# faltiska/Matcha-TTS-24k

Hardware: AMD Instinct MI355X
Metric: mel-frames/s (100-bin, 24 kHz) end-to-end synthesise(), n_timesteps=10 (higher is better)
Workload: dtype f32 via 2-term f16 split (fp32 accumulate); 1 GPU; configs[1]: batch=32 random phoneme seqs len=128, n_spks=1, euler n_timesteps=10, fp32, prod v20 architecture, random-init weights, T_pad=640 / 320 valid frames per utterance (reference 2x padding kept in the results; the estimator folds the identical padded frames, DESIGN.md section 4), noise from the device seed-42 generator; per_gpu_batch=32, global_batch=32, parallelism=dp1, n_feats=100

## Files before the change

### include/mtts.h

```cpp
#ifndef MTTS_H
#define MTTS_H

#include <stddef.h>
#include <stdint.h>

#ifdef __cplusplus
extern "C" {
#endif

#define MTTS_ABI_VERSION 2
#define MTTS_IMAGE_REVISION 6

typedef struct mtts_ctx mtts_ctx;

typedef struct mtts_config {
    int32_t n_feats;
    int32_t n_spks;
    int32_t spk_emb_dim;
    int32_t n_vocab;
    int32_t enc_channels;
    int32_t enc_filter;
    int32_t enc_heads;
    int32_t enc_layers;
    int32_t enc_kernel;
// ... 74 lines not shown
                  int a_nparts, const float* d_w,
                  void* d_wpacked, const float* d_bias, int N, int act, const float* d_p0, const float* d_p1,
                  const float* d_res, int ldr, const float* d_out_mask, float out_scale, float* d_out, int ldc,
                  float* d_stats_out, int terms, void* stream);

int64_t mtts_gemm_p16_scratch_bytes(int B, int T_in, int C, int T_out, int N);
int mtts_gemm_p16(const float* d_a, int lda, int B, int T_in, int C, int ntaps, const int* h_tap_off, int in_stride, int T_out,
                  const float* d_a_mask, const float* d_a_mean, const float* d_a_rstd, const float* d_a_part, int a_nparts,
                  const float* d_w, void* d_wpacked, const float* d_bias, int N, int act, const float* d_p0, const float* d_p1,
                  const float* d_res, int ldr, const float* d_out_mask, float out_scale, float* d_out, int ldc,
                  float* d_out16_f32, float out_lscale, float* d_stats_out, int force_bm, void* d_scratch, void* stream);

int64_t mtts_conv_gn_scratch_bytes(int B, int T, int C, int N);
int mtts_conv_gn(const float* d_x, int B, int T, int C, int c1, const float* d_w, void* d_wpacked, const float* d_bias, int N,
                 const float* d_gamma, const float* d_beta, const float* d_mask, const float* d_chbias, const int* d_nrows,
                 const int* d_nextra, const float* d_bias_stats, float eps, float* d_out, void* d_scratch, void* stream);

int mtts_attention_f32(const float* d_qkv, const float* d_mask, int B, int T, int H, int D, float scale, int mask_mode,
                       float* d_out, void* stream);

int mtts_attention_p16(const float* d_qkv, const float* d_mask, int B, int T, int H, int D, float scale, int mask_mode,
                       float* d_out, void* d_scratch, void* stream);

int64_t mtts_chain_stream_frags(int C, int inner, int ch, int n_qkv);
int mtts_chain_plan(int M, int ch, int* qb, int* prefetch_wgs);
int mtts_chain_stream_pack(int C, int inner, int ch, int n_qkv, const float* h_w_out, const float* h_w1, const float* h_w2,
                           const float* h_w_qkv, uint16_t* h_dst);
int64_t mtts_chain_stream_frags_pair(int C, int inner, int ch, int n_qkv);
int mtts_chain_stream_pack_pair(int C, int inner, int ch, int n_qkv, const float* h_w_out, const float* h_w1, const float* h_w2,
                                const float* h_w_qkv, uint16_t* h_dst);
int64_t mtts_tblock_chain_scratch_bytes(int M, int C, int inner, int n_qkv, int ch);
int mtts_tblock_chain(const float* d_att, const float* d_x, int M, int C, int inner, const float* h_w_out, const float* h_b_out,
                      const float* h_w1, const float* h_b1, const float* h_p0, const float* h_p1, const float* h_w2,
                      const float* h_b2, const float* h_w_qkv, const float* h_b_qkv, int n_qkv, const float* d_out_mask, int qb,
                      int ch, float* d_x_out, float* d_qkv_out, void* d_scratch, void* stream);
int mtts_tblock_chain_timed(const float* d_att, const float* d_x, int M, int C, int inner, const float* h_w_out, const float* h_b_out,
                            const float* h_w1, const float* h_b1, const float* h_p0, const float* h_p1, const float* h_w2,
                            const float* h_b2, const float* h_w_qkv, const float* h_b_qkv, int n_qkv, const float* d_out_mask,
                            int qb, int ch, float* d_x_out, float* d_qkv_out, void* d_scratch, void* stream, int repeat, float* h_ms);
int mtts_tblock_chain_pair_timed(const float* d_att, const float* d_x, int M, int C, int inner, const float* h_w_out, const float* h_b_out,
                                 const float* h_w1, const float* h_b1, const float* h_p0, const float* h_p1, const float* h_w2,
                                 const float* h_b2, const float* h_w_qkv, const float* h_b_qkv, int n_qkv, const float* d_out_mask,
                                 int qb, int ch, float* d_x_out, float* d_qkv_out, void* d_scratch, void* stream, int repeat, float* h_ms);

int64_t mtts_chain_stream_frags_h16(int C, int inner, int ch, int n_qkv);
int mtts_chain_stream_pack_h16(int C, int inner, int ch, int n_qkv, const float* h_w_out, const float* h_w1, const float* h_w2,
// ... 90 lines not shown
```

### matcha-tts-24k_amd/_hip.py

```python
from __future__ import annotations

import ctypes as C
import os
import subprocess
from pathlib import Path
from typing import Dict, Optional

import numpy as np
import torch

from .hparams import PathHParams

HERE = Path(__file__).resolve().parent
CSRC = HERE / "csrc"
LIB = Path(os.environ["MTTS_HIP_LIB"]) if os.environ.get("MTTS_HIP_LIB") else HERE / "libmtts_hip.so"
SOURCES = ["gemm_f32.hip", "attention_f32.hip", "gemm_p16.hip", "tblock_chain.hip", "tblock_chain_h16.hip", "resnet_conv.hip", "norm_glue.hip", "vocos.hip", "waveform.hip", "mel_frontend.hip", "style_encoder.hip", "mas.hip", "model.hip", "pack.hip", "decoder.hip", "encoder.hip", "unit_entries.hip"]
HEADERS = [CSRC / "kernels.h", CSRC / "device_utils.h", CSRC / "model.h", CSRC / "host.h", HERE.parent / "include" / "mtts.h"]
SOLVERS = {"euler": 0, "midpoint": 1, "rk4": 2}


class MttsConfig(C.Structure):
    _fields_ = [(n, C.c_int32) for n in (
        "n_feats", "n_spks", "spk_emb_dim", "n_vocab", "enc_channels", "enc_filter", "enc_heads", "enc_layers",
        "enc_kernel", "prenet_layers", "prenet_kernel", "dp_filter", "dp_kernel", "dp_layers", "dec_levels")] + [
# ... 87 lines not shown
        "mtts_import_weights": (i32, [vp, vp, i64, i32]),
        "mtts_encoder_workspace_bytes": (i64, [vp, i32, i32]),
        "mtts_text_encoder_forward": (i32, [vp, vp, vp, vp, vp, i32, i32, vp, vp, vp, vp, i64, vp]),
        "mtts_speaker_embedding": (i32, [vp, i32, vp, i32, vp, vp]),
        "mtts_durations": (i32, [vp, vp, f32, f32, i32, i32, vp, vp, vp, vp]),
        "mtts_durations_per_utterance": (i32, [vp, vp, vp, vp, i32, i32, vp, vp, vp, vp]),
        "mtts_durations_given": (i32, [vp, vp, f32, vp, vp, i32, i32, vp, vp, vp, vp]),
        "mtts_align_pool": (i32, [vp, vp, vp, i32, i32, i32, i32, vp, vp, vp, vp]),
        "mtts_set_frame_limits": (i32, [vp, vp]),
        "mtts_decoder_workspace_bytes": (i64, [vp, i32, i32]),
        "mtts_decoder_forward": (i32, [vp, vp, vp, vp, f32, i32, i32, vp, vp, i64, vp]),
        "mtts_cfm_solve": (i32, [vp, vp, vp, vp, i32, vp, i32, i32, i32, i32, vp, i32, f32, f32, vp, i64, vp]),
        "mtts_fold_rows": (i32, [vp, i32, i32]),
        "mtts_cfm_solve_folded": (i32, [vp, vp, vp, vp, i32, i32, vp, i32, i32, i32, i32, i32, vp, i32, f32, f32, vp, i64, vp]),
        "mtts_gemm_packed_bytes": (i64, [i32, i32, i32]),
        "mtts_attention_p16": (i32, [vp, vp, i32, i32, i32, i32, f32, i32, vp, vp, vp]),
        "mtts_gemm_p16_scratch_bytes": (i64, [i32, i32, i32, i32, i32]),
        "mtts_conv_gn_scratch_bytes": (i64, [i32, i32, i32, i32]),
        "mtts_conv_gn": (i32, [vp, i32, i32, i32, i32, vp, vp, vp, i32, vp, vp, vp, vp, vp, vp, vp, f32, vp, vp, vp]),
        "mtts_gemm_p16": (i32, [vp, i32, i32, i32, i32, i32, vp, i32, i32, vp, vp, vp, vp, i32, vp, vp, vp, i32, i32, vp, vp, vp,
                                i32, vp, f32, vp, i32, vp, f32, vp, i32, vp, vp]),
        "mtts_gemm_f32": (i32, [vp, i32, i32, i32, i32, i32, vp, i32, i32, vp, vp, vp, vp, i32, vp, vp, vp, i32, i32, vp, vp, vp,
                                i32, vp, f32, vp, i32, vp, i32, vp]),
        "mtts_attention_f32": (i32, [vp, vp, i32, i32, i32, i32, f32, i32, vp, vp]),
        "mtts_chain_stream_frags": (i64, [i32, i32, i32, i32]),
        "mtts_chain_plan": (i32, [i32, i32, C.POINTER(C.c_int), C.POINTER(C.c_int)]),
        "mtts_chain_stream_frags_pair": (i64, [i32, i32, i32, i32]),
        "mtts_chain_stream_pack_pair": (i32, [i32, i32, i32, i32, vp, vp, vp, vp, vp]),
        "mtts_chain_stream_pack": (i32, [i32, i32, i32, i32, vp, vp, vp, vp, vp]),
        "mtts_tblock_chain_scratch_bytes": (i64, [i32, i32, i32, i32, i32]),
        "mtts_tblock_chain": (i32, [vp, vp, i32, i32, i32, vp, vp, vp, vp, vp, vp, vp, vp, vp, vp, i32, vp, i32, i32, vp, vp, vp, vp]),
        "mtts_tblock_chain_timed": (i32, [vp, vp, i32, i32, i32, vp, vp, vp, vp, vp, vp, vp, vp, vp, vp, i32, vp, i32, i32, vp, vp, vp, vp,
                                          i32, C.POINTER(C.c_float)]),
        "mtts_tblock_chain_pair_timed": (i32, [vp, vp, i32, i32, i32, vp, vp, vp, vp, vp, vp, vp, vp, vp, vp, i32, vp, i32, i32, vp, vp, vp, vp,
                                          i32, C.POINTER(C.c_float)]),
        "mtts_chain_stream_frags_h16": (i64, [i32, i32, i32, i32]),
        "mtts_chain_stream_pack_h16": (i32, [i32, i32, i32, i32, vp, vp, vp, vp, i32, vp, C.POINTER(C.c_int)]),
        "mtts_tblock_chain_h16_scratch_bytes": (i64, [i32, i32, i32, i32, i32]),
        "mtts_tblock_chain_h16": (i32, [vp, vp, i32, i32, i32, vp, vp, vp, vp, vp, vp, vp, vp, vp, vp, i32, vp, i32, i32, i32, i32, vp, vp, vp, vp]),
        "mtts_tblock_chain_h16_timed": (i32, [vp, vp, i32, i32, i32, vp, vp, vp, vp, vp, vp, vp, vp, vp, vp, i32, vp, i32, i32, i32, i32, vp, vp, vp, vp,
                                              i32, C.POINTER(C.c_float)]),
        "mtts_row_stats": (i32, [vp, i32, i32, i32, f32, vp, vp, vp]),
        "mtts_channel_layernorm": (i32, [vp, i32, i32, i32, vp, vp, f32, i32, vp, vp, vp, vp]),
        "mtts_groupnorm_scratch_bytes": (i64, [i32, i32, i32]),
        "mtts_groupnorm_mish": (i32, [vp, vp, vp, vp, i32, i32, i32, i32, f32, vp, vp, vp]),
        "mtts_vocos_create": (vp, [i32, i32, i32, i32, i32, i32]),
# ... 599 lines not shown
                                          n_qkv, ptr(out_mask), int(bool(bf16)), qb, ch, pf_wgs, ptr(x_out), ptr(qkv), scratch.data_ptr(),
                                          stream_ptr(), repeat, C.byref(ms)))
    torch.cuda.synchronize()
    if repeat:
        return x_out, qkv, ms.value
    return x_out, qkv


def attention_f32(qkv, mask, B, T, H, D, scale, mask_mode):
    lib = load()
    out = torch.empty(B * T, H * D, dtype=torch.float32, device=qkv.device)
    check(lib.mtts_attention_f32(ptr(qkv), ptr(mask), B, T, H, D, float(scale), mask_mode, ptr(out), stream_ptr()))
    return out


def attention_p16(qkv, mask, B, T, H, D, scale, mask_mode):
    lib = load()
    out = torch.empty(B * T, H * D, dtype=torch.float32, device=qkv.device)
    scratch = torch.empty(16 * B * T * H * D, dtype=torch.uint8, device=qkv.device)
    check(lib.mtts_attention_p16(ptr(qkv), ptr(mask), B, T, H, D, float(scale), mask_mode, ptr(out), scratch.data_ptr(), stream_ptr()))
    return out


def row_stats(x, eps=1e-5):
    lib = load()
    M, Cc = x.shape
    mean = torch.empty(M, dtype=torch.float32, device=x.device)
    rstd = torch.empty(M, dtype=torch.float32, device=x.device)
    check(lib.mtts_row_stats(ptr(x), M, Cc, Cc, eps, ptr(mean), ptr(rstd), stream_ptr()))
    return mean, rstd


def channel_layernorm(x, gamma, beta, B, T, *, act=0, film=None, mask=None, eps=1e-5):
    lib = load()
    y = torch.empty_like(x)
    check(lib.mtts_channel_layernorm(ptr(x), B, T, x.shape[1], ptr(gamma), ptr(beta), float(eps), act, ptr(film), ptr(mask), ptr(y),
                                     stream_ptr()))
    return y


def groupnorm_mish(y, gamma, beta, mask, B, T, G=8, eps=1e-5):
    lib = load()
    Cc = y.shape[1]
    scratch = torch.empty(lib.mtts_groupnorm_scratch_bytes(B, T, G), dtype=torch.uint8, device=y.device)
    out = torch.empty_like(y)
    check(lib.mtts_groupnorm_mish(ptr(y), ptr(gamma), ptr(beta), ptr(mask), B, T, Cc, G, eps, ptr(out), scratch.data_ptr(),
# ... 3 lines not shown
```

### matcha-tts-24k_amd/csrc/attention_f32.hip

```cpp
#include "kernels.h"
#include "device_utils.h"
#include <cstdlib>
#include <string>

namespace mtts {

using f32x16 = __attribute__((ext_vector_type(16))) float;
using f32x4 = __attribute__((ext_vector_type(4))) float;
using f16x8 = __attribute__((ext_vector_type(8))) _Float16;
using f16x4 = __attribute__((ext_vector_type(4))) _Float16;

constexpr int AT_QW = 32;
constexpr int AT_K = 64;
constexpr int AT_D = 64;
constexpr int AT_KS = 72;
constexpr float NEG_BIG = -1e30f;
constexpr float LOG2E = 1.44269504088896340736f;

__device__ __forceinline__ f16x4 tr_read4(const _Float16* lds_ptr) {
    typedef __fp16 h4 __attribute__((__vector_size__(4 * sizeof(__fp16))));
    const h4 v = __builtin_amdgcn_ds_read_tr16_b64_v4f16((__attribute__((address_space(3))) h4*)(lds_ptr));
    return __builtin_bit_cast(f16x4, v);
}

using bf16x8_a = __attribute__((ext_vector_type(8))) __bf16;
template <bool BF>
__device__ __forceinline__ f32x16 att_mfma(f16x8 a, f16x8 b, f32x16 c) {
    if constexpr (BF) return __builtin_amdgcn_mfma_f32_32x32x16_bf16(__builtin_bit_cast(bf16x8_a, a), __builtin_bit_cast(bf16x8_a, b), c, 0, 0, 0);
    else return __builtin_amdgcn_mfma_f32_32x32x16_f16(a, b, c, 0, 0, 0);
}
template <int NW, bool P16, bool ONE = false, bool HALF = false, bool BF = false, int KR = AT_K>
__global__ __launch_bounds__(64 * NW, KR > AT_K ? 1 : 2) void attention_f32_kernel(const AttnArgs p) {
    static_assert(!HALF || (P16 && ONE), "H16 I/O runs the single-product loop");
    static_assert(!BF || HALF, "bfloat16 planes exist in the 16-bit storage mode only");
    constexpr bool WHOLE = KR > AT_K;
    constexpr int NT = 64 * NW;
    constexpr int SROWS = NT / 4;
    constexpr int SP = KR / SROWS;
    static_assert(SP >= 1 && SP * SROWS == KR && (!WHOLE || NW * AT_QW >= KR), "staging passes cover the rows held");
    __shared__ __attribute__((aligned(16))) _Float16 Ks[2 * KR * AT_KS];
    __shared__ __attribute__((aligned(16))) _Float16 Vs[2 * 2 * KR * 32];
    __shared__ __attribute__((aligned(16))) float Bs[KR];

    const int tid = threadIdx.x, lane = tid & 63, wave = tid >> 6;
    const int lq = lane & 31, h = lane >> 5;
    const int qblocks = (p.T + NW * AT_QW - 1) / (NW * AT_QW);
    int swz;
    {
        const int nwg = gridDim.x, id = blockIdx.x;
        const int xcd = id & 7, q = nwg >> 3, r = nwg & 7;
        swz = (xcd < r ? xcd * (q + 1) : r * (q + 1) + (xcd - r) * q) + (id >> 3);
    }
    const int qb = swz % qblocks, head = (swz / qblocks) % p.H, b = swz / (qblocks * p.H);
    const int q0 = qb * (NW * AT_QW) + wave * AT_QW;
    const int ld = 3 * p.H * p.D;
    const size_t rowbase = (size_t)b * p.T;
    const int Tb = p.klen ? min(p.T, p.klen[b]) : p.T;
    const float* qptr = p.qkv + head * p.D;
    const float* kptr = p.qkv + p.H * p.D + head * p.D;
    const float* vptr = p.qkv + 2 * p.H * p.D + head * p.D;
    const float ninf = -__builtin_huge_valf();

    const int qi = q0 + lq;
    const bool q_in = qi < p.T;
    const float scale2 = p.scale * LOG2E;
    f16x8 qh[4], ql[4];
    const _Float16* q16 = p.qkv16 + head * ((HALF ? 1 : 2) * AT_D);
    const _Float16* k16 = q16 + (HALF ? 1 : 2) * p.H * AT_D;
    const _Float16* v16 = q16 + (HALF ? 2 : 4) * p.H * AT_D;
    if constexpr (P16) {
        const _Float16* qrow = q16 + (rowbase + (q_in ? qi : 0)) * (size_t)p.ld16;
#pragma unroll
        for (int kb = 0; kb < 4; ++kb) {
            const f16x8 z = {0, 0, 0, 0, 0, 0, 0, 0};
            const _Float16* src = HALF ? qrow + 16 * kb + 8 * h : qrow + (kb >> 1) * 64 + (kb & 1) * 16 + 8 * h;
            qh[kb] = q_in ? *reinterpret_cast<const f16x8*>(src) : z;
            ql[kb] = (q_in && !HALF) ? *reinterpret_cast<const f16x8*>(src + 32) : z;
        }
    } else
#pragma unroll
    for (int kb = 0; kb < 4; ++kb) {
#pragma unroll
        for (int half4 = 0; half4 < 2; ++half4) {
            f32x4 v = {0.f, 0.f, 0.f, 0.f};
            const int d = 16 * kb + 8 * h + 4 * half4;
            if (q_in && d < p.D) v = *reinterpret_cast<const f32x4*>(qptr + (rowbase + qi) * ld + d);
#pragma unroll
            for (int e = 0; e < 4; ++e) {
                const _Float16 a = (_Float16)v[e];
                qh[kb][4 * half4 + e] = a;
                ql[kb][4 * half4 + e] = (_Float16)(v[e] - (float)a);
            }
        }
    }

    f32x16 o[2];
#pragma unroll
    for (int t = 0; t < 2; ++t)
#pragma unroll
        for (int r = 0; r < 16; ++r) o[t][r] = 0.f;
    float m_run = NEG_BIG, l_run = 0.f;

    const int srow = tid >> 2;
    const int sd = (tid & 3) * 4;
    f32x4 rk[SP][4], rv[SP][4];
    float rbias[SP];
    bool r_in[SP];
    auto fetch = [&](int k0) {
#pragma unroll
        for (int sp = 0; sp < SP; ++sp) {
            const int key = k0 + srow + SROWS * sp;
            r_in[sp] = key < Tb;
            const size_t row = rowbase + (r_in[sp] ? key : 0);
#pragma unroll
            for (int c = 0; c < 4; ++c) {
                if constexpr (HALF) {
                    if (c < 2) {
                        rk[sp][c] = *reinterpret_cast<const f32x4*>(k16 + row * p.ld16 + ((tid & 3) + 4 * c) * 8);
// ... 48 lines not shown
                *reinterpret_cast<f16x4*>(Ks + r * AT_KS + sd + 16 * c) = kh;
                *reinterpret_cast<f16x4*>(Ks + KR * AT_KS + r * AT_KS + sd + 16 * c) = kl;
                const f32x4 vv = ok ? rv[sp][c] : zero;
                f16x4 vh4, vl4;
#pragma unroll
                for (int e = 0; e < 4; ++e) {
                    const _Float16 a = (_Float16)vv[e];
                    vh4[e] = a;
                    vl4[e] = (_Float16)(vv[e] - (float)a);
                }
                const int dcol = sd + 16 * c;
                *reinterpret_cast<f16x4*>(Vs + ((dcol >> 5) * KR + r) * 32 + (dcol & 31)) = vh4;
                *reinterpret_cast<f16x4*>(Vs + ((2 + (dcol >> 5)) * KR + r) * 32 + (dcol & 31)) = vl4;
            }
            if ((tid & 3) == 0) {
                float bv = ninf;
                if (r_in[sp]) bv = (p.mask_mode == 0) ? rbias[sp] * LOG2E : (rbias[sp] != 0.f ? 0.f : ninf);
                Bs[r] = bv;
            }
        }
    };

    const int ntiles = (Tb + AT_K - 1) / AT_K;
    fetch(0);
    if constexpr (WHOLE) {
        stage();
        __syncthreads();
    }
    for (int kt = 0; kt < ntiles; ++kt) {
        const int kbase = WHOLE ? kt * AT_K : 0;
        if constexpr (!WHOLE) {
            if (kt) __syncthreads();
            stage();
            __syncthreads();
            if (kt + 1 < ntiles) fetch((kt + 1) * AT_K);
        }

        f32x16 s[2];
#pragma unroll
        for (int t = 0; t < 2; ++t) {
#pragma unroll
            for (int r = 0; r < 16; ++r) s[t][r] = 0.f;
            const _Float16* kp = Ks + (kbase + 32 * t + lq) * AT_KS + 8 * h;
#pragma unroll
            for (int kb = 0; kb < 4; ++kb) {
                const f16x8 kh = *reinterpret_cast<const f16x8*>(kp + 16 * kb);
                const f16x8 kl = *reinterpret_cast<const f16x8*>(kp + KR * AT_KS + 16 * kb);
                if constexpr (!ONE) {
                    s[t] = __builtin_amdgcn_mfma_f32_32x32x16_f16(kl, qh[kb], s[t], 0, 0, 0);
                    s[t] = __builtin_amdgcn_mfma_f32_32x32x16_f16(kh, ql[kb], s[t], 0, 0, 0);
                }
                s[t] = att_mfma<BF>(kh, qh[kb], s[t]);
            }
        }
        float mx = NEG_BIG;
#pragma unroll
        for (int t = 0; t < 2; ++t)
#pragma unroll
            for (int g4 = 0; g4 < 4; ++g4) {
                const f32x4 bb = *reinterpret_cast<const f32x4*>(Bs + kbase + 32 * t + 8 * g4 + 4 * h);
#pragma unroll
                for (int e = 0; e < 4; ++e) {
                    const float v = fmaf(s[t][4 * g4 + e], scale2, bb[e]);
                    s[t][4 * g4 + e] = v;
                    mx = fmaxf(mx, v);
                }
            }
        mx = fmaxf(mx, __shfl_xor(mx, 32));
        const float m_new = fmaxf(m_run, mx);
        const float alpha = __builtin_amdgcn_exp2f(m_run - m_new);
        float psum = 0.f;
#pragma unroll
        for (int t = 0; t < 2; ++t)
#pragma unroll
            for (int r = 0; r < 16; ++r) {
                const float pv = __builtin_amdgcn_exp2f(s[t][r] - m_new);
                s[t][r] = pv;
                psum += pv;
            }
        l_run = l_run * alpha + psum;
        if (__any(m_new != m_run)) {
#pragma unroll
            for (int t = 0; t < 2; ++t)
#pragma unroll
                for (int r = 0; r < 16; ++r) o[t][r] *= alpha;
        }
        m_run = m_new;
#pragma unroll
        for (int t = 0; t < 2; ++t)
#pragma unroll
            for (int ks = 0; ks < 2; ++ks) {
                f16x8 ph, pl;
                if constexpr (BF) {
                    using u32x4 = __attribute__((ext_vector_type(4))) unsigned int;
                    u32x4 w;
#pragma unroll
                    for (int j = 0; j < 4; ++j) w[j] = pack_bf16(s[t][8 * ks + 2 * j], s[t][8 * ks + 2 * j + 1]);
                    ph = __builtin_bit_cast(f16x8, w);
                    pl = ph;
                } else {
#pragma unroll
                    for (int j = 0; j < 8; ++j) {
                        const float pv = s[t][8 * ks + j];
                        const _Float16 a = (_Float16)pv;
                        ph[j] = a;
                        pl[j] = (_Float16)(pv - (float)a);
                    }
                }
                const int k0 = 32 * t + 16 * ks + 4 * h;
#pragma unroll
                for (int dt = 0; dt < 2; ++dt) {
                    const _Float16* vp = Vs + ((dt * KR) + kbase + k0 + ((lane & 15) >> 2)) * 32 + 16 * ((lane >> 4) & 1) + 4 * (lane & 3);
                    f16x8 vh, vl;
                    const f16x4 h0 = tr_read4(vp), h1 = tr_read4(vp + 8 * 32);
                    const f16x4 l0 = tr_read4(vp + 2 * KR * 32), l1 = tr_read4(vp + 2 * KR * 32 + 8 * 32);
#pragma unroll
                    for (int e = 0; e < 4; ++e) { vh[e] = h0[e]; vh[4 + e] = h1[e]; vl[e] = l0[e]; vl[4 + e] = l1[e]; }
                    if constexpr (!ONE) {
                        o[dt] = __builtin_amdgcn_mfma_f32_32x32x16_f16(vl, ph, o[dt], 0, 0, 0);
                        o[dt] = __builtin_amdgcn_mfma_f32_32x32x16_f16(vh, pl, o[dt], 0, 0, 0);
                    }
                    o[dt] = att_mfma<BF>(vh, ph, o[dt]);
                }
            }
    }

    const float l_tot = l_run + __shfl_xor(l_run, 32);
    const float inv = l_tot > 0.f ? 1.0f / l_tot : 0.f;
    bool range_bad = false;
    if (P16) {
        if (q_in) {
            _Float16* op = p.out16 + (rowbase + qi) * (size_t)p.ldo16 + head * ((HALF ? 1 : 2) * AT_D);
#pragma unroll
            for (int t = 0; t < 2; ++t)
#pragma unroll
                for (int g4 = 0; g4 < 4; ++g4) {
                    f16x4 hh, ll;
                    if constexpr (BF) {
                        using u32x2 = __attribute__((ext_vector_type(2))) unsigned int;
                        *reinterpret_cast<u32x2*>(op + t * 32 + 8 * g4 + 4 * h) =
                            u32x2{pack_bf16(o[t][4 * g4] * inv, o[t][4 * g4 + 1] * inv), pack_bf16(o[t][4 * g4 + 2] * inv, o[t][4 * g4 + 3] * inv)};
                        continue;
                    }
                    range_bad |= out_of_f16_range(o[t][4 * g4] * inv, o[t][4 * g4 + 1] * inv, o[t][4 * g4 + 2] * inv, o[t][4 * g4 + 3] * inv);
#pragma unroll
                    for (int e = 0; e < 4; ++e) {
                        _Float16 a, b;
// ... 29 lines not shown
    const bool p16 = a.qkv16 != nullptr;
    const int ew = a.half16 ? 1 : 2;
    if ((a.half16 && !p16) || (a.bf16 && !a.half16)) return hipErrorInvalidValue;
    if (p16 ? (!a.out16 || a.D != AT_D || a.ld16 < 3 * ew * a.H * AT_D || (a.ld16 & 7) || a.ldo16 < ew * a.H * AT_D || (a.ldo16 & 3))
            : (!a.qkv || !a.out))
        return hipErrorInvalidValue;
    if (a.B <= 0 || a.T <= 0 || a.H <= 0) return hipErrorInvalidValue;
    if (a.D <= 0 || a.D > AT_D || (a.D & 3)) return hipErrorInvalidValue;
    if (a.mask_mode == 1 && !a.mask) return hipErrorInvalidValue;
    const int b128 = (a.T + 127) / 128, b64 = (a.T + 63) / 64;
    const long blocks128 = (long)b128 * a.H * a.B;
    const double waste128 = 1.0 - (double)a.T / (b128 * 128.0);
    const bool same_rows = b128 * 128 == b64 * 64 && blocks128 >= 512;
    const bool use128 = (blocks128 >= 768 && waste128 < 0.1) || same_rows;
    {
        static thread_local std::string tag;
        const bool one = a.half16 || (p16 && a.fast16);
        tag = std::string("attention_f32_kernel<") + (use128 ? "4" : "2") + ", " + tf(p16) + ", " + tf(one) + ", " + tf(a.half16) + ", " + tf(a.half16 && a.bf16) + ", 64>";
        g_kernel_tag = tag.c_str();
    }
    if (p16 && a.T > 64 && a.T <= 192) {
        static thread_local std::string wtag;
        const bool one = a.half16 || a.fast16;
        wtag = std::string("attention_f32_kernel<6, true, ") + tf(one) + ", " + tf(a.half16) + ", " + tf(a.half16 && a.bf16) + ", 192>";
        g_kernel_tag = wtag.c_str();
        const dim3 grid(a.H * a.B), block(384);
        if (a.half16 && a.bf16) hipLaunchKernelGGL((attention_f32_kernel<6, true, true, true, true, 192>), grid, block, 0, s, a);
        else if (a.half16) hipLaunchKernelGGL((attention_f32_kernel<6, true, true, true, false, 192>), grid, block, 0, s, a);
        else if (a.fast16) hipLaunchKernelGGL((attention_f32_kernel<6, true, true, false, false, 192>), grid, block, 0, s, a);
        else hipLaunchKernelGGL((attention_f32_kernel<6, true, false, false, false, 192>), grid, block, 0, s, a);
        return hipGetLastError();
    }
    if (use128) {
        if (a.half16 && a.bf16) hipLaunchKernelGGL((attention_f32_kernel<4, true, true, true, true>), dim3(b128 * a.H * a.B), dim3(256), 0, s, a);
        else if (a.half16) hipLaunchKernelGGL((attention_f32_kernel<4, true, true, true>), dim3(b128 * a.H * a.B), dim3(256), 0, s, a);
        else if (p16 && a.fast16) hipLaunchKernelGGL((attention_f32_kernel<4, true, true>), dim3(b128 * a.H * a.B), dim3(256), 0, s, a);
        else if (p16) hipLaunchKernelGGL((attention_f32_kernel<4, true>), dim3(b128 * a.H * a.B), dim3(256), 0, s, a);
        else hipLaunchKernelGGL((attention_f32_kernel<4, false>), dim3(b128 * a.H * a.B), dim3(256), 0, s, a);
    } else {
        if (a.half16 && a.bf16) hipLaunchKernelGGL((attention_f32_kernel<2, true, true, true, true>), dim3(b64 * a.H * a.B), dim3(128), 0, s, a);
        else if (a.half16) hipLaunchKernelGGL((attention_f32_kernel<2, true, true, true>), dim3(b64 * a.H * a.B), dim3(128), 0, s, a);
        else if (p16 && a.fast16) hipLaunchKernelGGL((attention_f32_kernel<2, true, true>), dim3(b64 * a.H * a.B), dim3(128), 0, s, a);
        else if (p16) hipLaunchKernelGGL((attention_f32_kernel<2, true>), dim3(b64 * a.H * a.B), dim3(128), 0, s, a);
        else hipLaunchKernelGGL((attention_f32_kernel<2, false>), dim3(b64 * a.H * a.B), dim3(128), 0, s, a);
    }
    return hipGetLastError();
}

}
```

### matcha-tts-24k_amd/csrc/decoder.hip

```cpp
#include "host.h"

namespace mtts {

static int one_round_prefetchers(int M, int qb, int want) {
    const int nwg = (M + qb - 1) / qb;
    if (nwg <= CHIP_CUS && nwg + want > CHIP_CUS) return (want >= 8 && nwg + 8 <= CHIP_CUS) ? 8 : 0;
    return want;
}
void chain_plan(int M, int ch, int qb_forced, int want, int* qb, int* pf) {
    const int qb_big = ch == 256 ? 48 : 64;
    const bool fits32 = (M + 31) / 32 + want <= CHIP_CUS;
    *qb = (qb_forced == 32 || qb_forced == qb_big) ? qb_forced : (fits32 ? 32 : qb_big);
    *pf = one_round_prefetchers(M, *qb, want);
}
static int run_chain(mtts_ctx* c, const ChainArgs& a0, hipStream_t s) {
    ChainArgs a = a0;
    a.range_flag = c->cur_flag;
    { int qb_unused = 0; chain_plan(a.M, a.ch, a.qb, c->sw.chain_pf, &qb_unused, &a.pf_wgs); }
    if (a.pair) a.pf_wgs = c->sw.chain_pf ? 16 : 0;
    LAUNCHB(c, 0, chain_flops(a), chain_bytes(a), s, launch_tblock_chain(a, s));
    return 0;
}
static void chain16_plan(int M, int C, int ch, int qb_forced, int want, int* qb, int* pf) {
    const bool tall = C == 384 && ch == 256;
// ... 272 lines not shown
    const bool fuse = (C % 64) == 0;
    float* x = d.stream(dst);
    auto layernorm_in = [&](GemmArgs& p) -> int {
        bind_in(d, p, 0, actv(d, x, C));
        if (fuse) { p.a_part = d.lnp; p.a_nparts = C / 64; return 0; }
        LAUNCH(c, 2, 0, s, launch_row_stats(x, M, C, C, 1e-5f, d.mean, d.rstd, s));
        p.a_mean = d.mean; p.a_rstd = d.rstd;
        return 0;
    };
    const bool chain = t.chain_frags > 0 && !t.chain_h16 && d.p16 && !c->half_now && M >= c->sw.chain_min_rows && (emit_stats ? t.chain_nqkv > 0 : true);
    const bool chain16 = t.chain_frags > 0 && t.chain_h16 && d.p16 && c->half_now && d.ew == 1 && M >= c->sw.chain16_min_rows &&
                         (emit_stats ? t.chain_nqkv > 0 : true);
    if (!d.qkv_ready) {
        GemmArgs q;
        panel_args(c, t.qkv, q); rows_plain(q, B, T);
        RET_IF(layernorm_in(q));
        bind_out(d, q, d.QKV, 3 * inner, nullptr, 1.0f);
        RET_IF(run_gemm(c, q, s));
    }
    d.qkv_ready = false;
    AttnArgs at;
    bind_attn(d, at, d.QKV, d.ATT, inner);
    at.mask = d.kb(lvl); at.B = B; at.T = T; at.H = g.dec_heads; at.D = g.dec_head_dim;
    at.scale = 1.0f / sqrtf((float)g.dec_head_dim); at.mask_mode = 0; at.klen = d.nr(lvl); at.fast16 = c->fast16;
    RET_IF(run_attn(c, at, s));
    const int tiles48 = (M + 47) / 48;
    const bool pair = !chain && !chain16 && c->sw.pair_on && t.chain_pair_frags > 0 && d.p16 && !c->half_now && d.pair_flag && M >= c->sw.pair_min_rows &&
                      16 * ((tiles48 + 7) / 8) + 16 <= CHIP_CUS && (emit_stats ? t.chain_nqkv > 0 : true);
    auto bind_chain = [&](auto& a, int ew) {
        a.M = M; a.C = C; a.inner = inner;
        a.att16 = image(d.ATT); a.ld_att = ew * inner;
        a.x16 = image(x); a.ld_x = ew * C;
        a.wstream = static_cast<decltype(a.wstream)>(static_cast<const void*>(W(c, t.chain))); a.stream_frags = t.chain_frags;
        a.consts = W(c, t.chain_consts);
        a.ld_out = ew * C;
        if (emit_stats) {
            const TBlockW& nx = c->dec.tb[t.next];
            a.b_qkv = W(c, nx.qkv.b); a.wsum_qkv = W(c, nx.qkv.wsum); a.n_qkv = nx.qkv.N;
            a.qkv16 = image(d.QKV); a.ld_qkv = ew * nx.qkv.N;
            a.x_out = image(x);
            d.qkv_ready = true;
        } else { a.x_out = image(dst); a.x_out_mask = d.mask[lvl]; }
        a.ch = t.chain_ch;
    };
    if (chain16) {
        ChainH16Args a;
        bind_chain(a, 1);
// ... 295 lines not shown
```

### matcha-tts-24k_amd/csrc/kernels.h

```cpp
#pragma once
#include <hip/hip_runtime.h>
#include <stdint.h>

namespace mtts {

constexpr int GEMM_BM = 128;
constexpr int GEMM_BN = 128;
constexpr int GEMM_BK = 32;
constexpr int MAX_TAPS = 7;

static inline int round_up(int x, int m) { return (x + m - 1) / m * m; }

constexpr int CHIP_CUS = 256;

extern thread_local const char* g_kernel_tag;
static inline const char* tf(bool b) { return b ? "true" : "false"; }

enum Act { ACT_NONE = 0, ACT_RELU = 1, ACT_SILU = 2, ACT_SNAKE = 3, ACT_GELU = 4 };

struct GemmArgs {
    const float* a0 = nullptr;
    const float* a1 = nullptr;
    int lda0 = 0, lda1 = 0;
    int c0 = 0, c1 = 0;
// ... 75 lines not shown
hipError_t launch_pack_weight(const float* w, int N, int C, int ntaps, float* dst, hipStream_t s);
void split_panel_host(const float* panel, size_t n, uint16_t* planes);
hipError_t launch_split_panel(const float* panel, size_t n, void* planes, hipStream_t s);
void split_panel_f16_host(const float* panel, size_t n, uint16_t* planes);
void panel_h16_host(const float* panel, size_t n, uint16_t* plane);
void panel_bf16_host(const float* panel, size_t n, uint16_t* plane);
hipError_t launch_split_panel_f16(const float* panel, size_t n, void* planes, hipStream_t s);

struct AttnArgs {
    const float* qkv = nullptr;
    const float* mask = nullptr;
    float* out = nullptr;
    int B = 0, T = 0, H = 0, D = 0;
    float scale = 1.0f;
    int mask_mode = 0;
    const _Float16* qkv16 = nullptr; int ld16 = 0;
    _Float16* out16 = nullptr; int ldo16 = 0;
    float out_lscale = 2048.0f;
    const int* klen = nullptr;
    bool fast16 = false;
    unsigned int* range_flag = nullptr;
    bool half16 = false;
    bool bf16 = false;
};
hipError_t launch_attention(const AttnArgs& a, hipStream_t s);
static inline double attn_flops(const AttnArgs& a) { return 4.0 * double(a.B) * a.H * double(a.T) * a.T * a.D; }
static inline double attn_bytes(const AttnArgs& a) { return 4.0 * double(a.B) * a.T * 4.0 * a.H * a.D; }

constexpr int CONV_GN_CPG = 48;
constexpr int CONV_GN_MIN_ROWS = 65;
constexpr int CONV_GN_SPLIT_ROWS = 192;
constexpr int CONV_GN_MAX_ROWS = 384;
struct ConvGnArgs {
    const _Float16* a16_0 = nullptr;
    const _Float16* a16_1 = nullptr;
    int lda16_0 = 0, lda16_1 = 0;
    int c0 = 0, c1 = 0;
    const void* w16 = nullptr;
    const float* bias = nullptr;
    int B = 0, T = 0, N = 0;
    const float* gamma = nullptr; const float* beta = nullptr;
    const float* mask = nullptr;
    const float* chbias = nullptr;
    const int* nrows = nullptr;
    const int* nextra = nullptr;
    const float* bias_stats = nullptr;
    float eps = 1e-5f;
// ... 210 lines not shown
```

### matcha-tts-24k_amd/csrc/model.h

```cpp
#pragma once
#include <atomic>
#include <map>
#include <string>
#include <vector>

#include "../../include/mtts.h"
#include "kernels.h"

namespace mtts {

void set_error(const std::string& msg);
const char* get_error();

struct Panel {
    size_t w = 0, b = 0;
    size_t w16 = 0;
    bool has_bias = false;
    size_t wsum = 0;
    size_t wh16 = 0;
    int N = 0, C = 0, ntaps = 1, ktap = 0;
};
struct Vec { size_t off = 0; int n = 0; };

struct ResnetW {
// ... 48 lines not shown
    std::vector<Vec> dw_w, dw_b, ln_g, ln_b;
    std::vector<Panel> pw1, pw2;
};

struct StyleW {
    std::vector<Panel> convs;
    Vec proj_w, proj_b;
};

struct Switches {
    int gemm_terms = 2;
    int arith16 = 0;
    bool p16_on = true;
    bool chain_on = true;
    int chain_ch = 256;
    int chain_qb = 0;
    int chain_min_rows = 5761;
    bool pair_on = true;
    int pair_min_rows = 3000;
    int chain_pf = 16;
    bool chain16_on = true;
    int chain16_min_rows = 5000;
    int chain16_qb = 0;
    int resnet_fuse = 3;
};
Switches read_switches();

struct ProfRec { hipEvent_t e0, e1; int klass; double flops, bytes; std::string tag; };

}

namespace mtts {
struct Component {
    std::map<std::string, std::vector<float>> raw;
    std::vector<float> image;
    float* d_image = nullptr;
    bool packed = false, uploaded = false;
    bool weights_saturate = false;
    int gemm_terms = 6;
    bool half16 = false;
    bool bf16 = false;
    bool fast16 = false;
    unsigned int* cur_flag = nullptr;
    bool half_now = false;
    bool prof_on = false;
    std::vector<ProfRec> prof;
// ... 30 lines not shown
```

### matcha-tts-24k_amd/csrc/model.hip

```cpp
#include "host.h"

#include <cstdlib>
#include <time.h>

namespace mtts {

static thread_local std::string g_err;
void set_error(const std::string& m) { g_err = m; }
const char* get_error() { return g_err.c_str(); }

Switches read_switches() {
    Switches w;
    auto num = [](const char* name, int dflt) { const char* e = getenv(name); return e ? atoi(e) : dflt; };
    auto on = [](const char* name) { const char* e = getenv(name); return !(e && e[0] == '0'); };
    const int terms = num("MTTS_GEMM_TERMS", w.gemm_terms);
    if (terms == 0 || terms == 2 || terms == 3 || terms == 6) w.gemm_terms = terms;
    if (terms == 1 || terms == 16 || terms == 17) w.arith16 = terms;
    w.p16_on = on("MTTS_P16");
    w.chain_on = on("MTTS_CHAIN");
    if (num("MTTS_CHAIN_CH", w.chain_ch) == 128) w.chain_ch = 128;
    w.chain_qb = num("MTTS_CHAIN_QB", w.chain_qb);
    w.chain_min_rows = num("MTTS_CHAIN_MIN_ROWS", w.chain_min_rows);
    w.pair_on = on("MTTS_CHAIN_PAIR");
    w.pair_min_rows = num("MTTS_CHAIN_PAIR_MIN_ROWS", w.pair_min_rows);
    w.chain_pf = std::min(std::max(num("MTTS_CHAIN_PF", w.chain_pf), 0), 64);
    w.chain16_on = on("MTTS_CHAIN16");
    w.chain16_min_rows = num("MTTS_CHAIN16_MIN_ROWS", w.chain16_min_rows);
    { const int qb = num("MTTS_CHAIN16_QB", 0); if (qb == 32 || qb == 64 || qb == 96) w.chain16_qb = qb; }
    w.resnet_fuse = num("MTTS_RESNET_FUSE", w.resnet_fuse) & 7;
    return w;
}

}

using namespace mtts;

static int pack_ctx(mtts_ctx* c) { return pack_all(c); }

extern "C" {

int mtts_abi_version(void) { return MTTS_ABI_VERSION; }
const char* mtts_last_error(void) { return get_error(); }

mtts_ctx* mtts_create(const mtts_config* cfg) {
    if (!cfg) { set_error("null config"); return nullptr; }
    const mtts_config& g = *cfg;
    std::string why;
    if (g.dec_levels < 1 || g.dec_levels > 4) why = "dec_levels must be 1..4";
    else if (g.n_feats <= 0 || (2 * g.n_feats) % 4) why = "n_feats must be even";
    else if ((g.enc_channels + g.spk_emb_dim) % g.enc_heads) why = "encoder hidden size not divisible by heads";
    else if (((g.enc_channels + g.spk_emb_dim) / g.enc_heads) % 4 || (g.enc_channels + g.spk_emb_dim) / g.enc_heads > 64) why = "encoder head dim must be a multiple of 4, <= 64";
// ... 153 lines not shown
```

### matcha-tts-24k_amd/csrc/unit_entries.hip

```cpp
#include "host.h"

using namespace mtts;

static double plain_row_sum(const float* w, int K, bool) {
    double a = 0.0;
    for (int k = 0; k < K; ++k) a += (double)w[k];
    return a;
}
static double rounded_row_sum(const float* w, int K, bool bf16) {
    double a = 0.0;
    for (int k = 0; k < K; ++k) a += bf16 ? (double)(float)(__bf16)w[k] : (double)(float)(_Float16)fminf(fmaxf(w[k], -65504.f), 65504.f);
    return a;
}
static std::vector<float> chain_entry_consts(int C, int inner, int n_qkv, const float* h_b_out, const float* h_w1, const float* h_b1,
                                             const float* h_p0, const float* h_p1, const float* h_b2, const float* h_w_qkv,
                                             const float* h_b_qkv, double (*row_sum)(const float*, int, bool), bool bf16) {
    std::vector<float> hc((size_t)18 * C + 2 * (size_t)n_qkv, 0.f);
    for (int n = 0; n < 4 * C; ++n) {
        hc[n] = (float)row_sum(h_w1 + (size_t)n * C, C, bf16);
        hc[4 * C + n] = h_b1 ? h_b1[n] : 0.f;
        hc[8 * C + n] = h_p0[n];
        hc[12 * C + n] = h_p1[n];
    }
    for (int n = 0; n < C; ++n) { hc[16 * C + n] = (inner && h_b_out) ? h_b_out[n] : 0.f; hc[17 * C + n] = h_b2 ? h_b2[n] : 0.f; }
// ... 173 lines not shown
                       void* stream) {
    AttnArgs a;
    a.qkv = d_qkv; a.mask = d_mask; a.out = d_out; a.B = B; a.T = T; a.H = H; a.D = D; a.scale = scale; a.mask_mode = mask_mode;
    HIP_OK(launch_attention(a, static_cast<hipStream_t>(stream)));
    return 0;
}

int mtts_attention_p16(const float* d_qkv, const float* d_mask, int B, int T, int H, int D, float scale, int mask_mode, float* d_out,
                       void* d_scratch, void* stream) {
    hipStream_t s = static_cast<hipStream_t>(stream);
    if (D != 64 || !d_scratch) { set_error("P16 attention needs D == 64 and a scratch buffer"); return -1; }
    const int M = B * T, C3 = 3 * H * D;
    _Float16* q16 = static_cast<_Float16*>(d_scratch);
    _Float16* o16 = q16 + (size_t)M * 2 * C3;
    HIP_OK(launch_to_p16(d_qkv, C3, nullptr, M, C3, C3, q16, 2 * C3, 1.0f, s));
    AttnArgs a;
    a.qkv16 = q16; a.ld16 = 2 * C3; a.out16 = o16; a.ldo16 = 2 * H * D; a.mask = d_mask;
    a.B = B; a.T = T; a.H = H; a.D = D; a.scale = scale; a.mask_mode = mask_mode;
    HIP_OK(launch_attention(a, s));
    HIP_OK(launch_from_p16(o16, 2 * H * D, M, H * D, a.out_lscale, d_out, H * D, s));
    return 0;
}

int mtts_row_stats(const float* d_x, int M, int C, int ld, float eps, float* d_mean, float* d_rstd, void* stream) {
    HIP_OK(launch_row_stats(d_x, M, C, ld, eps, d_mean, d_rstd, static_cast<hipStream_t>(stream)));
    return 0;
}

int mtts_channel_layernorm(const float* d_x, int B, int T, int C, const float* d_gamma, const float* d_beta, float eps, int act,
                           const float* d_film, const float* d_mask, float* d_y, void* stream) {
    if (B <= 0 || T <= 0) { set_error("mtts_channel_layernorm: empty batch"); return -1; }
    if (act != ACT_NONE && act != ACT_SILU) { set_error("mtts_channel_layernorm: act must be 0 (none) or 2 (SiLU)"); return -1; }
    LayerNormArgs a;
    a.x = d_x; a.ldx = C; a.y = d_y; a.ldy = C; a.M = B * T; a.C = C; a.T = T; a.gamma = d_gamma; a.beta = d_beta; a.eps = eps;
    a.act = act; a.film = d_film; a.mask = d_mask;
    HIP_OK(launch_layernorm(a, static_cast<hipStream_t>(stream)));
    return 0;
}

int64_t mtts_groupnorm_scratch_bytes(int B, int T, int G) { return (int64_t)B * gn_chunks_max(T) * G * 2 * (int64_t)sizeof(float); }

int mtts_groupnorm_mish(const float* d_y, const float* d_gamma, const float* d_beta, const float* d_mask, int B, int T, int C, int G,
                        float eps, float* d_out, void* d_scratch, void* stream) {
    hipStream_t s = static_cast<hipStream_t>(stream);
    HIP_OK(launch_gn_partial(d_y, B, T, C, G, static_cast<float*>(d_scratch), s));
    GnApplyArgs a;
// ... 157 lines not shown
```

Baseline: 445,300 mel-frames/s.

## Add split-key and fine-tile attention variants with LDS-resident low Q half

Adds two attention kernel forms selected by a new switch. The default (form 2) routes short sequences through a 4-wave, 64-key tile variant that keeps the low half of Q in LDS to cut register pressure (allowing 3 blocks per CU), skips compute for idle waves past T, and runs a half-width final tile. Form 1 splits the whole-K path across twice as many waves, each doing half the keys, then merges softmax partials through LDS. It also adds a test entry point; the change risks extra LDS traffic and a sync for the merge.

Result: no change. 444,500 mel-frames/s (median of 4 runs) (-0.2%).

```diff
diff --git a/include/mtts.h b/include/mtts.h
--- a/include/mtts.h
+++ b/include/mtts.h
@@ -120,6 +120,9 @@
 int mtts_attention_p16(const float* d_qkv, const float* d_mask, int B, int T, int H, int D, float scale, int mask_mode,
                        float* d_out, void* d_scratch, void* stream);
 
+int mtts_attention_forms(const float* d_qkv, const float* d_bias, const int* d_klen, int B, int T, int H, float scale, int form, int arith,
+                         float* d_out, float* d_in, void* d_scratch, void* stream);
+
 int64_t mtts_chain_stream_frags(int C, int inner, int ch, int n_qkv);
 int mtts_chain_plan(int M, int ch, int* qb, int* prefetch_wgs);
 int mtts_chain_stream_pack(int C, int inner, int ch, int n_qkv, const float* h_w_out, const float* h_w1, const float* h_w2,
diff --git a/matcha-tts-24k_amd/_hip.py b/matcha-tts-24k_amd/_hip.py
--- a/matcha-tts-24k_amd/_hip.py
+++ b/matcha-tts-24k_amd/_hip.py
@@ -133,6 +133,7 @@
                                 i32, vp, f32, vp, i32, vp, f32, vp, i32, vp, vp]),
         "mtts_gemm_f32": (i32, [vp, i32, i32, i32, i32, i32, vp, i32, i32, vp, vp, vp, vp, i32, vp, vp, vp, i32, i32, vp, vp, vp,
                                 i32, vp, f32, vp, i32, vp, i32, vp]),
+        "mtts_attention_forms": (i32, [vp, vp, vp, i32, i32, i32, f32, i32, i32, vp, vp, vp, vp]),
         "mtts_attention_f32": (i32, [vp, vp, i32, i32, i32, i32, f32, i32, vp, vp]),
         "mtts_chain_stream_frags": (i64, [i32, i32, i32, i32]),
         "mtts_chain_plan": (i32, [i32, i32, C.POINTER(C.c_int), C.POINTER(C.c_int)]),
@@ -778,6 +779,17 @@
     return out
 
 
+def attention_forms(qkv, bias, klen, B, T, H, scale, form, arith=2, want_inputs=False):
+    lib = load()
+    D = 64
+    out = torch.empty(B * T, H * D, dtype=torch.float32, device=qkv.device)
+    seen = torch.empty(B * T, 3 * H * D, dtype=torch.float32, device=qkv.device) if want_inputs else None
+    scratch = torch.empty(16 * B * T * H * D, dtype=torch.uint8, device=qkv.device)
+    check(lib.mtts_attention_forms(ptr(qkv), ptr(bias), ptr(klen) if klen is not None else None, B, T, H, float(scale), form, arith,
+                                   ptr(out), ptr(seen) if want_inputs else None, scratch.data_ptr(), stream_ptr()))
+    return (out, seen) if want_inputs else out
+
+
 def row_stats(x, eps=1e-5):
     lib = load()
     M, Cc = x.shape
diff --git a/matcha-tts-24k_amd/csrc/attention_f32.hip b/matcha-tts-24k_amd/csrc/attention_f32.hip
--- a/matcha-tts-24k_amd/csrc/attention_f32.hip
+++ b/matcha-tts-24k_amd/csrc/attention_f32.hip
@@ -2,6 +2,7 @@
 #include "device_utils.h"
 #include <cstdlib>
 #include <string>
+#include <type_traits>
 
 namespace mtts {
 
@@ -29,22 +30,28 @@
     if constexpr (BF) return __builtin_amdgcn_mfma_f32_32x32x16_bf16(__builtin_bit_cast(bf16x8_a, a), __builtin_bit_cast(bf16x8_a, b), c, 0, 0, 0);
     else return __builtin_amdgcn_mfma_f32_32x32x16_f16(a, b, c, 0, 0, 0);
 }
-template <int NW, bool P16, bool ONE = false, bool HALF = false, bool BF = false, int KR = AT_K>
-__global__ __launch_bounds__(64 * NW, KR > AT_K ? 1 : 2) void attention_f32_kernel(const AttnArgs p) {
+template <int NW, bool P16, bool ONE = false, bool HALF = false, bool BF = false, int KR = AT_K, bool NF = false>
+__global__ __launch_bounds__(64 * NW, NF ? 3 : (KR > AT_K ? 1 : 2)) void attention_f32_kernel(const AttnArgs p) {
     static_assert(!HALF || (P16 && ONE), "H16 I/O runs the single-product loop");
     static_assert(!BF || HALF, "bfloat16 planes exist in the 16-bit storage mode only");
+    static_assert(!NF || P16, "the new forms read P16 / H16 images");
     constexpr bool WHOLE = KR > AT_K;
+    constexpr bool SPLIT = WHOLE && NF;
+    constexpr int QW = SPLIT ? NW / 2 : NW;
     constexpr int NT = 64 * NW;
     constexpr int SROWS = NT / 4;
     constexpr int SP = KR / SROWS;
-    static_assert(SP >= 1 && SP * SROWS == KR && (!WHOLE || NW * AT_QW >= KR), "staging passes cover the rows held");
+    static_assert(SP >= 1 && SP * SROWS == KR && (!WHOLE || QW * AT_QW >= KR), "staging passes cover the rows held");
     __shared__ __attribute__((aligned(16))) _Float16 Ks[2 * KR * AT_KS];
     __shared__ __attribute__((aligned(16))) _Float16 Vs[2 * 2 * KR * 32];
     __shared__ __attribute__((aligned(16))) float Bs[KR];
+    constexpr bool QL_LDS = NF && !WHOLE && !ONE;
+    __shared__ __attribute__((aligned(16))) _Float16 Qls[QL_LDS ? NW * AT_QW * AT_KS : 8];
+    __shared__ float Xs[SPLIT ? QW * 34 * 64 : 1];
 
     const int tid = threadIdx.x, lane = tid & 63, wave = tid >> 6;
     const int lq = lane & 31, h = lane >> 5;
-    const int qblocks = (p.T + NW * AT_QW - 1) / (NW * AT_QW);
+    const int qblocks = (p.T + QW * AT_QW - 1) / (QW * AT_QW);
     int swz;
     {
         const int nwg = gridDim.x, id = blockIdx.x;
@@ -52,10 +59,11 @@
         swz = (xcd < r ? xcd * (q + 1) : r * (q + 1) + (xcd - r) * q) + (id >> 3);
     }
     const int qb = swz % qblocks, head = (swz / qblocks) % p.H, b = swz / (qblocks * p.H);
-    const int q0 = qb * (NW * AT_QW) + wave * AT_QW;
+    const int qwave = (SPLIT && wave >= QW) ? wave - QW : wave;
+    const int q0 = qb * (QW * AT_QW) + qwave * AT_QW;
     const int ld = 3 * p.H * p.D;
     const size_t rowbase = (size_t)b * p.T;
-    const int Tb = p.klen ? min(p.T, p.klen[b]) : p.T;
+    const int Tb = p.klen ? max(0, min(p.T, p.klen[b])) : p.T;
     const float* qptr = p.qkv + head * p.D;
     const float* kptr = p.qkv + p.H * p.D + head * p.D;
     const float* vptr = p.qkv + 2 * p.H * p.D + head * p.D;
@@ -94,6 +102,12 @@
         }
     }
 
+    const _Float16* qlp = Qls + (wave * AT_QW + lq) * AT_KS + 8 * h;
+    if constexpr (QL_LDS) {
+#pragma unroll
+        for (int kb = 0; kb < 4; ++kb) *reinterpret_cast<f16x8*>(Qls + (wave * AT_QW + lq) * AT_KS + 8 * h + 16 * kb) = ql[kb];
+    }
+
     f32x16 o[2];
 #pragma unroll
     for (int t = 0; t < 2; ++t)
@@ -188,23 +202,11 @@
     };
 
     const int ntiles = (Tb + AT_K - 1) / AT_K;
-    fetch(0);
-    if constexpr (WHOLE) {
-        stage();
-        __syncthreads();
-    }
-    for (int kt = 0; kt < ntiles; ++kt) {
-        const int kbase = WHOLE ? kt * AT_K : 0;
-        if constexpr (!WHOLE) {
-            if (kt) __syncthreads();
-            stage();
-            __syncthreads();
-            if (kt + 1 < ntiles) fetch((kt + 1) * AT_K);
-        }
-
-        f32x16 s[2];
-#pragma unroll
-        for (int t = 0; t < 2; ++t) {
+    auto tile = [&](auto ns, const int kbase) __attribute__((always_inline)) {
+        constexpr int NS = decltype(ns)::value;
+        f32x16 s[NS];
+#pragma unroll
+        for (int t = 0; t < NS; ++t) {
 #pragma unroll
             for (int r = 0; r < 16; ++r) s[t][r] = 0.f;
             const _Float16* kp = Ks + (kbase + 32 * t + lq) * AT_KS + 8 * h;
@@ -214,14 +216,17 @@
                 const f16x8 kl = *reinterpret_cast<const f16x8*>(kp + KR * AT_KS + 16 * kb);
                 if constexpr (!ONE) {
                     s[t] = __builtin_amdgcn_mfma_f32_32x32x16_f16(kl, qh[kb], s[t], 0, 0, 0);
-                    s[t] = __builtin_amdgcn_mfma_f32_32x32x16_f16(kh, ql[kb], s[t], 0, 0, 0);
+                    f16x8 qlk;
+                    if constexpr (QL_LDS) qlk = *reinterpret_cast<const f16x8*>(qlp + 16 * kb);
+                    else qlk = ql[kb];
+                    s[t] = __builtin_amdgcn_mfma_f32_32x32x16_f16(kh, qlk, s[t], 0, 0, 0);
                 }
                 s[t] = att_mfma<BF>(kh, qh[kb], s[t]);
             }
         }
         float mx = NEG_BIG;
 #pragma unroll
-        for (int t = 0; t < 2; ++t)
+        for (int t = 0; t < NS; ++t)
 #pragma unroll
             for (int g4 = 0; g4 < 4; ++g4) {
                 const f32x4 bb = *reinterpret_cast<const f32x4*>(Bs + kbase + 32 * t + 8 * g4 + 4 * h);
@@ -237,7 +242,7 @@
         const float alpha = __builtin_amdgcn_exp2f(m_run - m_new);
         float psum = 0.f;
 #pragma unroll
-        for (int t = 0; t < 2; ++t)
+        for (int t = 0; t < NS; ++t)
 #pragma unroll
             for (int r = 0; r < 16; ++r) {
                 const float pv = __builtin_amdgcn_exp2f(s[t][r] - m_new);
@@ -253,7 +258,7 @@
         }
         m_run = m_new;
 #pragma unroll
-        for (int t = 0; t < 2; ++t)
+        for (int t = 0; t < NS; ++t)
 #pragma unroll
             for (int ks = 0; ks < 2; ++ks) {
                 f16x8 ph, pl;
@@ -289,6 +294,65 @@
                     o[dt] = att_mfma<BF>(vh, ph, o[dt]);
                 }
             }
+    };
+    using one_sub = std::integral_constant<int, 1>;
+    using two_subs = std::integral_constant<int, 2>;
+    fetch(0);
+    if constexpr (WHOLE) {
+        stage();
+        __syncthreads();
+    }
+    if constexpr (SPLIT) {
+        const int n32 = (Tb + AT_QW - 1) / AT_QW, nlo = (n32 + 1) >> 1;
+        int st = wave < QW ? 0 : nlo;
+        const int s1 = wave < QW ? nlo : n32;
+        for (; st + 2 <= s1; st += 2) tile(two_subs{}, st * AT_QW);
+        if (st < s1) tile(one_sub{}, st * AT_QW);
+        float* xs = Xs + qwave * (34 * 64) + lane;
+        if (wave >= QW) {
+            xs[0] = m_run;
+            xs[64] = l_run;
+#pragma unroll
+            for (int t = 0; t < 2; ++t)
+#pragma unroll
+                for (int r = 0; r < 16; ++r) xs[(2 + 16 * t + r) * 64] = o[t][r];
+        }
+        __syncthreads();
+        if (wave >= QW) return;
+        {
+            const float m_b = xs[0], l_b = xs[64];
+            const float m_new = fmaxf(m_run, m_b);
+            const float fa = __builtin_amdgcn_exp2f(m_run - m_new), fb = __builtin_amdgcn_exp2f(m_b - m_new);
+            l_run = l_run * fa + l_b * fb;
+#pragma unroll
+            for (int t = 0; t < 2; ++t)
+#pragma unroll
+                for (int r = 0; r < 16; ++r) o[t][r] = o[t][r] * fa + xs[(2 + 16 * t + r) * 64] * fb;
+            m_run = m_new;
+        }
+    } else if constexpr (WHOLE) {
+        for (int kt = 0; kt < ntiles; ++kt) tile(two_subs{}, kt * AT_K);
+    } else {
+        const bool idle = NF && q0 >= p.T;
+        const int nfull = NF ? (Tb >> 6) + ((Tb & 63) > AT_QW ? 1 : 0) : ntiles;
+        auto advance = [&](int kt) {
+            if (kt) __syncthreads();
+            stage();
+            __syncthreads();
+            if (kt + 1 < ntiles) fetch((kt + 1) * AT_K);
+        };
+        if (idle) {
+            for (int kt = 0; kt < ntiles; ++kt) advance(kt);
+        } else {
+            for (int kt = 0; kt < nfull; ++kt) {
+                advance(kt);
+                tile(two_subs{}, 0);
+            }
+            if (nfull < ntiles) {
+                advance(nfull);
+                tile(one_sub{}, 0);
+            }
+        }
     }
 
     const float l_tot = l_run + __shfl_xor(l_run, 32);
@@ -364,13 +428,32 @@
     if (p16 && a.T > 64 && a.T <= 192) {
         static thread_local std::string wtag;
         const bool one = a.half16 || a.fast16;
-        wtag = std::string("attention_f32_kernel<6, true, ") + tf(one) + ", " + tf(a.half16) + ", " + tf(a.half16 && a.bf16) + ", 192>";
+        const bool split = a.form & 1;
+        wtag = std::string("attention_f32_kernel<") + (split ? "12" : "6") + ", true, " + tf(one) + ", " + tf(a.half16) + ", " + tf(a.half16 && a.bf16) + ", 192" + (split ? ", true>" : ">");
         g_kernel_tag = wtag.c_str();
-        const dim3 grid(a.H * a.B), block(384);
-        if (a.half16 && a.bf16) hipLaunchKernelGGL((attention_f32_kernel<6, true, true, true, true, 192>), grid, block, 0, s, a);
+        const dim3 grid(a.H * a.B), block(split ? 768 : 384);
+        if (split) {
+            if (a.half16 && a.bf16) hipLaunchKernelGGL((attention_f32_kernel<12, true, true, true, true, 192, true>), grid, block, 0, s, a);
+            else if (a.half16) hipLaunchKernelGGL((attention_f32_kernel<12, true, true, true, false, 192, true>), grid, block, 0, s, a);
+            else if (a.fast16) hipLaunchKernelGGL((attention_f32_kernel<12, true, true, false, false, 192, true>), grid, block, 0, s, a);
+            else hipLaunchKernelGGL((attention_f32_kernel<12, true, false, false, false, 192, true>), grid, block, 0, s, a);
+        }
+        else if (a.half16 && a.bf16) hipLaunchKernelGGL((attention_f32_kernel<6, true, true, true, true, 192>), grid, block, 0, s, a);
         else if (a.half16) hipLaunchKernelGGL((attention_f32_kernel<6, true, true, true, false, 192>), grid, block, 0, s, a);
         else if (a.fast16) hipLaunchKernelGGL((attention_f32_kernel<6, true, true, false, false, 192>), grid, block, 0, s, a);
         else hipLaunchKernelGGL((attention_f32_kernel<6, true, false, false, false, 192>), grid, block, 0, s, a);
+        return hipGetLastError();
+    }
+    if (p16 && use128 && (a.form & 2) && a.T <= ATTN_FINE_MAX_T) {
+        static thread_local std::string ftag;
+        const bool one = a.half16 || a.fast16;
+        ftag = std::string("attention_f32_kernel<4, true, ") + tf(one) + ", " + tf(a.half16) + ", " + tf(a.half16 && a.bf16) + ", 64, true>";
+        g_kernel_tag = ftag.c_str();
+        const dim3 grid(b128 * a.H * a.B), block(256);
+        if (a.half16 && a.bf16) hipLaunchKernelGGL((attention_f32_kernel<4, true, true, true, true, AT_K, true>), grid, block, 0, s, a);
+        else if (a.half16) hipLaunchKernelGGL((attention_f32_kernel<4, true, true, true, false, AT_K, true>), grid, block, 0, s, a);
+        else if (a.fast16) hipLaunchKernelGGL((attention_f32_kernel<4, true, true, false, false, AT_K, true>), grid, block, 0, s, a);
+        else hipLaunchKernelGGL((attention_f32_kernel<4, true, false, false, false, AT_K, true>), grid, block, 0, s, a);
         return hipGetLastError();
     }
     if (use128) {
diff --git a/matcha-tts-24k_amd/csrc/decoder.hip b/matcha-tts-24k_amd/csrc/decoder.hip
--- a/matcha-tts-24k_amd/csrc/decoder.hip
+++ b/matcha-tts-24k_amd/csrc/decoder.hip
@@ -318,7 +318,7 @@
     AttnArgs at;
     bind_attn(d, at, d.QKV, d.ATT, inner);
     at.mask = d.kb(lvl); at.B = B; at.T = T; at.H = g.dec_heads; at.D = g.dec_head_dim;
-    at.scale = 1.0f / sqrtf((float)g.dec_head_dim); at.mask_mode = 0; at.klen = d.nr(lvl); at.fast16 = c->fast16;
+    at.scale = 1.0f / sqrtf((float)g.dec_head_dim); at.mask_mode = 0; at.klen = d.nr(lvl); at.fast16 = c->fast16; at.form = c->sw.attn;
     RET_IF(run_attn(c, at, s));
     const int tiles48 = (M + 47) / 48;
     const bool pair = !chain && !chain16 && c->sw.pair_on && t.chain_pair_frags > 0 && d.p16 && !c->half_now && d.pair_flag && M >= c->sw.pair_min_rows &&
diff --git a/matcha-tts-24k_amd/csrc/kernels.h b/matcha-tts-24k_amd/csrc/kernels.h
--- a/matcha-tts-24k_amd/csrc/kernels.h
+++ b/matcha-tts-24k_amd/csrc/kernels.h
@@ -121,7 +121,9 @@
     unsigned int* range_flag = nullptr;
     bool half16 = false;
     bool bf16 = false;
-};
+    int form = 2;
+};
+constexpr int ATTN_FINE_MAX_T = 512;
 hipError_t launch_attention(const AttnArgs& a, hipStream_t s);
 static inline double attn_flops(const AttnArgs& a) { return 4.0 * double(a.B) * a.H * double(a.T) * a.T * a.D; }
 static inline double attn_bytes(const AttnArgs& a) { return 4.0 * double(a.B) * a.T * 4.0 * a.H * a.D; }
diff --git a/matcha-tts-24k_amd/csrc/model.h b/matcha-tts-24k_amd/csrc/model.h
--- a/matcha-tts-24k_amd/csrc/model.h
+++ b/matcha-tts-24k_amd/csrc/model.h
@@ -94,6 +94,7 @@
     bool chain16_on = true;
     int chain16_min_rows = 5000;
     int chain16_qb = 0;
+    int attn = 2;
     int resnet_fuse = 3;
 };
 Switches read_switches();
diff --git a/matcha-tts-24k_amd/csrc/model.hip b/matcha-tts-24k_amd/csrc/model.hip
--- a/matcha-tts-24k_amd/csrc/model.hip
+++ b/matcha-tts-24k_amd/csrc/model.hip
@@ -27,6 +27,7 @@
     w.chain16_on = on("MTTS_CHAIN16");
     w.chain16_min_rows = num("MTTS_CHAIN16_MIN_ROWS", w.chain16_min_rows);
     { const int qb = num("MTTS_CHAIN16_QB", 0); if (qb == 32 || qb == 64 || qb == 96) w.chain16_qb = qb; }
+    w.attn = num("MTTS_ATTN", w.attn) & 3;
     w.resnet_fuse = num("MTTS_RESNET_FUSE", w.resnet_fuse) & 7;
     return w;
 }
diff --git a/matcha-tts-24k_amd/csrc/unit_entries.hip b/matcha-tts-24k_amd/csrc/unit_entries.hip
--- a/matcha-tts-24k_amd/csrc/unit_entries.hip
+++ b/matcha-tts-24k_amd/csrc/unit_entries.hip
@@ -219,6 +219,30 @@
     return 0;
 }
 
+int mtts_attention_forms(const float* d_qkv, const float* d_bias, const int* d_klen, int B, int T, int H, float scale, int form, int arith,
+                         float* d_out, float* d_in, void* d_scratch, void* stream) {
+    hipStream_t s = static_cast<hipStream_t>(stream);
+    if (!d_scratch || (arith != 1 && arith != 2 && arith != 16 && arith != 17)) { set_error("mtts_attention_forms: arith must be 1, 2, 16 or 17"); return -1; }
+    const bool half16 = arith >= 16, bf16 = arith == 17;
+    const int M = B * T, D = 64, C3 = 3 * H * D, ew = half16 ? 1 : 2;
+    _Float16* q16 = static_cast<_Float16*>(d_scratch);
+    _Float16* o16 = q16 + (size_t)M * 2 * C3;
+    HIP_OK(launch_to_p16(d_qkv, C3, nullptr, M, C3, C3, q16, ew * C3, 1.0f, s, nullptr, half16, bf16));
+    AttnArgs a;
+    a.qkv16 = q16; a.ld16 = ew * C3; a.out16 = o16; a.ldo16 = ew * H * D; a.mask = d_bias; a.klen = d_klen;
+    a.B = B; a.T = T; a.H = H; a.D = D; a.scale = scale; a.mask_mode = 0;
+    a.fast16 = arith == 1; a.half16 = half16; a.bf16 = bf16; a.form = form;
+    HIP_OK(launch_attention(a, s));
+    if (half16) {
+        HIP_OK(launch_from_h16(o16, H * D, M, H * D, bf16, d_out, H * D, s));
+        if (d_in) HIP_OK(launch_from_h16(q16, C3, M, C3, bf16, d_in, C3, s));
+    } else {
+        HIP_OK(launch_from_p16(o16, 2 * H * D, M, H * D, a.out_lscale, d_out, H * D, s));
+        if (d_in) HIP_OK(launch_from_p16(q16, 2 * C3, M, C3, 1.0f, d_in, C3, s));
+    }
+    return 0;
+}
+
 int mtts_row_stats(const float* d_x, int M, int C, int ld, float eps, float* d_mean, float* d_rstd, void* stream) {
     HIP_OK(launch_row_stats(d_x, M, C, ld, eps, d_mean, d_rstd, static_cast<hipStream_t>(stream)));
     return 0;
```
